# kartikmadhira1/YA_VO

Measured on AMD Instinct MI355X. Metric: frames/sec (detect+describe+match+PnP) on 1241×376 KITTI stereo; RMSE vs CPU ref, higher is better.
Workload: dtype u8

## Files before the change

ya_vo_amd/csrc/yavo_batch.hip:

```cpp
#include "yavo_host.h"

using namespace yavo;

namespace {

constexpr int kMaxTimedRuns = 4096;

int upload_pairs_rev(yv_batch* b) {
    if (!b->m2_alloc || b->n_pairs <= 0) return YV_OK;
    std::vector<int32_t> r(b->h_pairs.size());
    for (size_t i = 0; i + 1 < r.size(); i += 2) {
        r[i] = b->h_pairs[i + 1];
        r[i + 1] = b->h_pairs[i];
    }
    YV_HIP(hipMemcpyAsync(b->pairs_rev, r.data(), sizeof(int32_t) * r.size(), hipMemcpyHostToDevice, b->ctx->stream));
    YV_HIP(hipStreamSynchronize(b->ctx->stream));
    return YV_OK;
}

int record_stage(yv_batch* b, hipStream_t s, int run, int stage) {
    if (!b->timing || run < 0) return YV_OK;
    if (b->timing == 2 && stage > 1) return YV_OK;
    YV_HIP(hipEventRecord(b->events[(size_t)run * kEvPerRun + stage], s));
    return YV_OK;
}

yavo::MatchLists match_lists(const yv_batch* b) { return {b->desc, b->keypoints, b->kp_count, b->max_kp}; }

yavo::MatchRecords match_records(const yv_batch* b, bool deferred) {
    return {b->matches,  b->match_count, b->filtered, b->filt_count,
            b->match_dj, b->match_lim,   deferred ? b->match_pos : nullptr};
}

int ensure_match_pos(yv_batch* b) {
    if (b->match_pos) return YV_OK;
    return b->mem.alloc(&b->match_pos, (size_t)std::max(b->max_pairs, 1) * (size_t)b->max_kp);
}

static_assert(YV_SUBPIX_NONE == yavo::kSubpixNone && YV_SUBPIX_OK == yavo::kSubpixOk &&
                  YV_SUBPIX_OUTSIDE == yavo::kSubpixOutside && YV_SUBPIX_EDGE == yavo::kSubpixEdge,
              "yavo.h / yavo_internal.h");

int subpix_fill_none(yv_batch* b, hipStream_t s) {
    const size_t n = (size_t)std::max(b->max_pairs, 1) * (size_t)b->max_kp;
    YV_HIP(hipMemsetAsync(b->subpix_dcol, 0, n * sizeof(int32_t), s));
    YV_HIP(hipMemsetAsync(b->subpix_sad, 0xFF, n * sizeof(int32_t), s));
    YV_HIP(hipMemsetAsync(b->subpix_status, YV_SUBPIX_NONE, n, s));
    return YV_OK;
}

int ensure_subpix(yv_batch* b) {
    if (b->subpix_alloc) return YV_OK;
    const size_t nk = (size_t)b->max_kp, np = (size_t)std::max(b->max_pairs, 1);
    int rc = YV_OK;
    rc |= b->mem.alloc(&b->subpix_pairs, np);
    rc |= b->mem.alloc(&b->subpix_dcol, np * nk);
    rc |= b->mem.alloc(&b->subpix_sad, np * nk);
    rc |= b->mem.alloc(&b->subpix_status, np * nk);
    if (rc != YV_OK) {
        b->mem.release(b->subpix_pairs, b->subpix_dcol, b->subpix_sad, b->subpix_status);
        return YV_ERR_HIP;
    }
    b->subpix_alloc = true;
    return YV_OK;
}

}

namespace yavo {

void batch_free(yv_batch* b) {
    if (!b) return;
    if (b->bstream) (void)hipStreamSynchronize(b->bstream);
    if (b->side) (void)hipStreamSynchronize(b->side);
    if (b->rstream) (void)hipStreamSynchronize(b->rstream);
    if (b->lk) yv_lk_destroy(b->lk);
    delete b;
}

static_assert(YV_MATCH_RATIO == yavo::kMatchRatio && YV_MATCH_MUTUAL == yavo::kMatchMutual, "yavo.h / yavo_internal.h");
static_assert(sizeof(yv_match2) == sizeof(int4), "nn2 is written as int4 {d1, j1, d2, j2}");

bool match_filter_args_ok(int flags, int num, int den) {
    if (flags < 0 || flags > (YV_MATCH_RATIO | YV_MATCH_MUTUAL)) return false;
    if ((flags & YV_MATCH_RATIO) && !(num > 0 && num <= den && den <= 32768)) return false;
    return true;
}

int ensure_match2(yv_batch* b) {
    if (b->m2_alloc) return YV_OK;
    const size_t nk = (size_t)b->max_kp, np = (size_t)std::max(b->max_pairs, 1);
    int rc = YV_OK;
    rc |= b->mem.alloc(&b->match_key2, np * nk);
    rc |= b->mem.alloc(&b->rev_key, np * nk);
    rc |= b->mem.alloc(&b->pairs_rev, np * 2);
    rc |= b->mem.alloc(&b->nn2, np * nk);
    rc |= b->mem.alloc(&b->rev, np * nk);
    rc |= b->mem.alloc(&b->keep, np * nk);
    if (rc != YV_OK) {
        b->mem.release(b->match_key2, b->rev_key, b->pairs_rev, b->nn2, b->rev, b->keep);
        return YV_ERR_HIP;
    }
    hipStream_t s = b->ctx->stream;
    YV_HIP(hipMemsetAsync(b->match_key2, 0xFF, np * nk * sizeof(uint32_t), s));
    YV_HIP(hipMemsetAsync(b->rev_key, 0xFF, np * nk * sizeof(uint32_t), s));
    YV_HIP(hipMemsetAsync(b->nn2, 0, np * nk * sizeof(int4), s));
    YV_HIP(hipMemsetAsync(b->rev, 0xFF, np * nk * sizeof(int32_t), s));
    YV_HIP(hipMemsetAsync(b->keep, 0, np * nk, s));
    YV_HIP(hipStreamSynchronize(s));
    b->m2_alloc = true;
    return upload_pairs_rev(b);
}

bool gate_ok(const int32_t* g) {
    for (int k = 0; k < 4; ++k)
        if (g[k] < -yavo::kGateMaxCoord || g[k] > yavo::kGateMaxCoord) return false;
    return g[0] <= g[1] && g[2] <= g[3];
}

int ensure_gates(yv_batch* b, int max_row, int max_col) {
    if (b->gate_alloc) return YV_OK;
    const int n_bands = max_row / yavo::kGateBandRows + 1;
    int shift = 6;
    while (n_bands * ((max_col >> shift) + 1) > yavo::kGateMaxCells && shift < 16) ++shift;
    if (n_bands * ((max_col >> shift) + 1) > yavo::kGateMaxCells) return YV_ERR_CAPACITY;
    const size_t nk = (size_t)b->max_kp, np = (size_t)std::max(b->max_pairs, 1), ns = (size_t)b->nslots;
    int rc = YV_OK;
    rc |= b->mem.alloc(&b->gates, np * 4);
    rc |= b->mem.alloc(&b->gate_sorted, ns * nk);
    rc |= b->mem.alloc(&b->gate_band, ns * (size_t)(n_bands + 1));
    if (rc != YV_OK) {
        b->mem.release(b->gates, b->gate_sorted, b->gate_band);
        return YV_ERR_HIP;
    }
    b->gate_bands = n_bands;
    b->gate_cols = (max_col >> shift) + 1;
    b->gate_shift = shift;
    b->gate_alloc = true;
    return YV_OK;
}

bool select_fits(const yv_ctx* ctx, int H, int W) {
    if (ctx->sel_q <= 0) return true;
    const int64_t cy = (H + ctx->sel_rows - 1) / ctx->sel_rows, cx = (W + ctx->sel_cols - 1) / ctx->sel_cols;
    return cy * cx <= yavo::kSelMaxCells;
}

int ensure_select(yv_batch* b) {
    if (b->sel_alloc) return YV_OK;
    const size_t ni = (size_t)b->max_images;
    int rc = YV_OK;
    rc |= b->mem.alloc(&b->sel_keys, ni * (size_t)b->cap);
    rc |= b->mem.alloc(&b->sel_starts, ni * (size_t)(yavo::kSelMaxCells + 1));
    rc |= b->mem.alloc(&b->sel_counts, 3 * ni);
    if (rc != YV_OK) {
        b->mem.release(b->sel_keys, b->sel_starts, b->sel_counts);
        return YV_ERR_HIP;
    }
    b->sel_alloc = true;
    return YV_OK;
}

void launch_select_topk(yv_batch* b, int n_images, int keep, hipStream_t s) {
    const yv_ctx* ctx = b->ctx;
    uint32_t* count = b->cand_count;
    uint32_t* seen = b->cand_seen;
    if (select_on(ctx)) {
        count = yavo::launch_select(b->cand_keys, b->cap, b->cand_count, b->cand_seen, n_images, b->H, b->W,
                                    ctx->sel_radius, ctx->sel_rows, ctx->sel_cols, ctx->sel_q, b->sel_keys,
                                    b->sel_starts, b->sel_counts, s);
        seen = b->sel_counts + 2 * (size_t)b->max_images;
    }
    yavo::launch_topk(b->cand_keys, b->cap, count, seen, n_images, b->H, b->W, b->max_kp, keep, b->det_rc, b->det_resp,
                      b->det_count, b->kp_src, b->kp_count, b->kp_band, b->band_off, b->brief_heads, s);
}

int ensure_steer(yv_batch* b) {
    if (b->steer_alloc) return YV_OK;
    const size_t n = (size_t)b->nslots * (size_t)b->max_kp;
    int rc = YV_OK;
    rc |= b->mem.alloc(&b->steer_bin, n);
    rc |= b->mem.alloc(&b->steer_mom, 2 * n);
    if (rc != YV_OK) {
        b->mem.release(b->steer_bin, b->steer_mom);
        return YV_ERR_HIP;
    }
    hipStream_t s = b->ctx->stream;
    YV_HIP(hipMemsetAsync(b->steer_bin, 0, n, s));
    YV_HIP(hipMemsetAsync(b->steer_mom, 0, 2 * n * sizeof(int32_t), s));
    YV_HIP(hipStreamSynchronize(s));
    b->steer_alloc = true;
    return YV_OK;
}

void launch_describe(yv_batch* b, int n_images, int max_workers, hipStream_t s) {
    yv_ctx* ctx = b->ctx;
    if (steer_on(ctx)) {
        const yavo::SteerTables t{ctx->steer_bins, ctx->steer_radius, ctx->d_steer_dirs, ctx->d_steer_addr};
        yavo::launch_brief_steer(b->blur, n_images, b->H, b->W, t, b->kp_src, b->kp_count, b->max_kp, b->keypoints,
                                 b->desc, b->steer_bin, b->steer_mom, s);
        return;
    }
    const bool new_loff = b->loff_version != ctx->offsets_version;
    b->loff_version = ctx->offsets_version;
    yavo::launch_brief(b->blur, n_images, b->H, b->W, ctx->d_offsets, b->kp_src, b->kp_band, b->band_off, b->max_kp,
                       b->keypoints, b->desc, b->brief_loff, new_loff, b->brief_heads, max_workers, s);
}

int prepare_select(yv_batch* b, int H, int W) {
    if (!select_on(b->ctx)) return YV_OK;
    if (!select_fits(b->ctx, H, W)) return YV_ERR_CAPACITY;
    return ensure_select(b);
}

int match_stage(yv_batch* b, MatchStage st, hipStream_t s, int run) {
    const yavo::MatchLists lists = match_lists(b);
    uint32_t* key2 = st.top2 ? b->match_key2 : nullptr;
    if (st.gated) {
        yavo::launch_gate_sort(b->keypoints, b->kp_count, b->nslots, b->max_kp, b->gate_bands, b->gate_cols,
                               b->gate_shift, b->gate_sorted, b->gate_band, s);
        yavo::launch_match_gated(lists, b->pairs, st.n_pairs, b->gate_bands, b->gate_sorted, b->gate_band, b->gates,
                                 false, b->match_key, key2, s);
        if (st.with_rev)
            yavo::launch_match_gated(lists, b->pairs_rev, st.n_pairs, b->gate_bands, b->gate_sorted, b->gate_band,
                                     b->gates, true, b->rev_key, nullptr, s);
    } else {
        yavo::launch_match(lists, b->pairs, st.n_pairs, st.max_train, b->match_key, key2, s);
        if (st.with_rev) yavo::launch_match(lists, b->pairs_rev, st.n_pairs, st.max_train_rev, b->rev_key, nullptr, s);
    }
    const int rc = record_stage(b, s, run, 4);
    const yavo::FinalizeRobust rb{b->match_key2, b->rev_key, st.flags, st.num, st.den, b->nn2, b->rev, b->keep};
    const yavo::MatchRecords out = match_records(b, st.defer_records);
    yavo::launch_match_finalize(b->match_key, lists, b->pairs, st.n_pairs, st.thr, out, st.top2 ? &rb : nullptr, s,
                                st.kp_count_copy, st.n_slots);
    if (st.defer_records) {
        YV_HIP(hipEventRecord(b->ev_keys, s));
        YV_HIP(hipStreamWaitEvent(b->rstream, b->ev_keys, 0));
        yavo::launch_match_records({lists.desc, lists.keypoints, st.kp_count_copy, lists.max_kp}, b->pairs, st.n_pairs,
                                   out, records_workgroups(b->ctx), b->rstream);
        YV_HIP(hipEventRecord(b->ev_records, b->rstream));
        b->records_pending = true;
    }
    return rc;
}

}

extern "C" {

int yv_batch_create(yv_ctx* ctx, int max_images, int H, int W, int max_kp, int max_pairs, yv_batch** out) {
    if (!ctx || !out || max_images <= 0 || H < 9 || W < 9 || max_kp <= 0 || max_kp > yavo::kMaxKp ||
        max_pairs < 0 || (int64_t)H * W >= (1ll << 31))
        return YV_ERR_INVALID;
    if (W > yavo::kMaxWidth) return YV_ERR_CAPACITY;
    if (H > yavo::kBandRows * yavo::kMaxBands) return YV_ERR_CAPACITY;
    *out = nullptr;
    if (set_device(ctx) != YV_OK) return YV_ERR_HIP;
    yv_batch* b = new (std::nothrow) yv_batch();
    if (!b) return YV_ERR_INVALID;
    b->ctx = ctx;
    b->max_images = max_images;
    b->H = H;
    b->W = W;
    b->max_kp = max_kp;
    b->max_pairs = max_pairs;
    b->nslots = max_images + 1;
    b->cap = (int64_t)(H - 8) * (W - 8);
    const size_t ns = (size_t)b->nslots, nk = (size_t)max_kp, np = (size_t)std::max(max_pairs, 1);
    int rc = YV_OK;
    rc |= b->mem.alloc(&b->cand_keys, (size_t)max_images * (size_t)b->cap);
    rc |= b->mem.alloc(&b->cand_count, ns);
    rc |= b->mem.alloc(&b->cand_seen, ns);
    rc |= b->mem.alloc(&b->det_rc, ns * nk * 2);
    rc |= b->mem.alloc(&b->det_resp, ns * nk);
    rc |= b->mem.alloc(&b->det_count, ns);
    rc |= b->mem.alloc(&b->kp_src, ns * nk * 4);
    rc |= b->mem.alloc(&b->kp_count, ns);
    rc |= b->mem.alloc(&b->kp_count_build, ns);
    rc |= b->mem.alloc(&b->kp_band, ns * nk * 4);
    rc |= b->mem.alloc(&b->band_off, ns * (size_t)(yavo::kMaxBands + 1));
    rc |= b->mem.alloc(&b->brief_loff, 512);
    rc |= b->mem.alloc(&b->brief_heads, (size_t)yavo::kBriefHeads);
    rc |= b->mem.alloc(&b->keypoints, ns * nk);
    rc |= b->mem.alloc(&b->desc, ns * nk);
    rc |= b->mem.alloc(&b->blur, (size_t)max_images * (size_t)yavo::blur_image_bytes(H, W));
    rc |= b->mem.alloc(&b->pairs, np * 2);
    rc |= b->mem.alloc(&b->match_key, np * nk);
    rc |= b->mem.alloc(&b->matches, np * nk);
    rc |= b->mem.alloc(&b->match_count, np);
    rc |= b->mem.alloc(&b->filtered, np * nk);
    rc |= b->mem.alloc(&b->filt_count, np);
    rc |= b->mem.alloc(&b->match_dj, np * nk);
    rc |= b->mem.alloc(&b->match_lim, np);
    rc |= b->mem.alloc(&b->staging, (size_t)H * W);
    if (rc != YV_OK) {
        batch_free(b);
        return YV_ERR_HIP;
    }
    hipStream_t s = ctx->stream;
    bool ok = hipMemsetAsync(b->cand_count, 0, ns * sizeof(uint32_t), s) == hipSuccess &&
              hipMemsetAsync(b->cand_seen, 0, ns * sizeof(uint32_t), s) == hipSuccess &&
              hipMemsetAsync(b->kp_count, 0, ns * sizeof(int32_t), s) == hipSuccess &&
              hipMemsetAsync(b->det_count, 0, ns * sizeof(int32_t), s) == hipSuccess &&
              hipMemsetAsync(b->match_key, 0xFF, np * nk * sizeof(uint32_t), s) == hipSuccess &&
              hipMemsetAsync(b->keypoints, 0, ns * nk * sizeof(yv_keypoint), s) == hipSuccess &&
              hipMemsetAsync(b->match_count, 0, np * sizeof(int32_t), s) == hipSuccess &&
              hipMemsetAsync(b->filt_count, 0, np * sizeof(int32_t), s) == hipSuccess &&
              hipMemsetAsync(b->match_lim, 0, np * sizeof(int32_t), s) == hipSuccess &&
              hipStreamSynchronize(s) == hipSuccess;
    if (!ok) {
        batch_free(b);
        return YV_ERR_HIP;
    }
    *out = b;
    return YV_OK;
}

void yv_batch_destroy(yv_batch* b) {
    if (!b) return;
    (void)hipSetDevice(b->ctx->device);
    (void)hipStreamSynchronize(b->ctx->stream);
    batch_free(b);
}

int yv_batch_set_pairs(yv_batch* b, const int32_t* pairs, int n_pairs) {
    if (!b || n_pairs < 0 || n_pairs > b->max_pairs || (n_pairs > 0 && !pairs)) return YV_ERR_INVALID;
    for (int i = 0; i < 2 * n_pairs; ++i)
        if (pairs[i] < 0 || pairs[i] > b->max_images) return YV_ERR_INVALID;
    if (set_device(b->ctx) != YV_OK) return YV_ERR_HIP;
    if (b->bstream) YV_HIP(hipStreamSynchronize(b->bstream));
    b->build_pending = false;
    if (drain_records(b) != YV_OK) return YV_ERR_HIP;
    if (n_pairs > 0) {
        YV_HIP(hipMemcpyAsync(b->pairs, pairs, sizeof(int32_t) * 2 * (size_t)n_pairs, hipMemcpyHostToDevice,
                              b->ctx->stream));
        YV_HIP(hipStreamSynchronize(b->ctx->stream));
    }
    b->h_pairs.assign(pairs, pairs + 2 * (size_t)n_pairs);
    b->n_pairs = n_pairs;
    b->n_tracks = 0;
    b->gated = false;
    b->subpix_on = false;
    return upload_pairs_rev(b);
}

int yv_batch_set_stereo_subpix(yv_batch* b, const int32_t* pair_idx, int n, int half_win, int search, int flags) {
    if (!b || n < 0) return YV_ERR_INVALID;
    if (!pair_idx || n == 0) {
        b->subpix_on = false;
        return YV_OK;
    }
    if (half_win < 1 || half_win > yavo::kSubpixMaxWin || search < 1 || search > yavo::kSubpixMaxSearch || flags < 0 ||
        flags > YV_SUBPIX_DROP_EDGE || n > b->n_pairs)
        return YV_ERR_INVALID;
    std::vector<uint8_t> seen((size_t)b->n_pairs, 0);
    for (int i = 0; i < n; ++i) {
        const int p = pair_idx[i];
        if (p < 0 || p >= b->n_pairs || seen[p]) return YV_ERR_INVALID;
        if (b->h_pairs[2 * p] >= b->max_images || b->h_pairs[2 * p + 1] >= b->max_images) return YV_ERR_INVALID;
        seen[p] = 1;
    }
    if (set_device(b->ctx) != YV_OK) return YV_ERR_HIP;
    const int rc = ensure_subpix(b);
    if (rc != YV_OK) return rc;
    hipStream_t s = b->ctx->stream;
    YV_HIP(hipDeviceSynchronize());
    b->build_pending = false;
    YV_HIP(hipMemcpyAsync(b->subpix_pairs, pair_idx, sizeof(int32_t) * (size_t)n, hipMemcpyHostToDevice, s));
    if (subpix_fill_none(b, s) != YV_OK) return YV_ERR_HIP;
    YV_HIP(hipStreamSynchronize(s));
    b->subpix_n = n;
    b->subpix_win = half_win;
    b->subpix_search = search;
    b->subpix_flags = flags;
    b->subpix_on = true;
    return YV_OK;
}

int yv_batch_subpix_view_get(yv_batch* b, yv_batch_subpix_view* v) {
    if (!b || !v || !b->subpix_alloc) return YV_ERR_INVALID;
    v->dcol_q8 = b->subpix_dcol;
    v->sad = b->subpix_sad;
    v->status = b->subpix_status;
    return YV_OK;
}

int yv_batch_set_match_gates(yv_batch* b, const int32_t* gates, int n_pairs) {
    if (!b) return YV_ERR_INVALID;
    if (!gates || n_pairs == 0) {
        b->gated = false;
        return YV_OK;
    }
    if (n_pairs != b->n_pairs) return YV_ERR_INVALID;
    for (int p = 0; p < n_pairs; ++p)
        if (!gate_ok(gates + 4 * p)) return YV_ERR_INVALID;
    if (set_device(b->ctx) != YV_OK) return YV_ERR_HIP;
    const int rc = ensure_gates(b, b->H - 1, b->W - 1);
    if (rc != YV_OK) return rc;
    YV_HIP(hipStreamSynchronize(b->ctx->stream));
    YV_HIP(hipMemcpyAsync(b->gates, gates, sizeof(int32_t) * 4 * (size_t)n_pairs, hipMemcpyHostToDevice,
                          b->ctx->stream));
    YV_HIP(hipStreamSynchronize(b->ctx->stream));
    b->gated = true;
    return YV_OK;
}

int yv_batch_set_match_filter(yv_batch* b, int flags, int ratio_num, int ratio_den) {
    if (!match_filter_args_ok(flags, ratio_num, ratio_den) || !b) return YV_ERR_INVALID;
    if (flags != 0) {
        if (set_device(b->ctx) != YV_OK) return YV_ERR_HIP;
        const int rc = ensure_match2(b);
        if (rc != YV_OK) return rc;
    }
    b->match_flags = flags;
    b->ratio_num = (flags & YV_MATCH_RATIO) ? ratio_num : 0;
    b->ratio_den = (flags & YV_MATCH_RATIO) ? ratio_den : 1;
    return YV_OK;
}

int yv_batch_match2_view_get(yv_batch* b, yv_batch_match2_view* v) {
    if (!b || !v || !b->m2_alloc) return YV_ERR_INVALID;
    v->nn2 = reinterpret_cast<const yv_match2*>(b->nn2);
    v->rev = b->rev;
    v->keep = b->keep;
    return YV_OK;
}

int yv_batch_orient_view_get(yv_batch* b, yv_batch_orient_view* v) {
    if (!b || !v || !b->steer_alloc) return YV_ERR_INVALID;
    v->bin = b->steer_bin;
    v->moments = b->steer_mom;
    return YV_OK;
}

int yv_batch_enable_timing(yv_batch* b, int on) {
    if (!b) return YV_ERR_INVALID;
    if (on && b->events.empty()) {
        if (set_device(b->ctx) != YV_OK) return YV_ERR_HIP;
        b->events.resize((size_t)kMaxTimedRuns * kEvPerRun);
        for (auto& e : b->events) YV_HIP(b->mem.event(&e, hipEventDefault));
        b->tracked.assign(kMaxTimedRuns, 0);
    }
    b->timing = on == 2 ? 2 : (on != 0 ? 1 : 0);
    b->runs_recorded = 0;
    b->last_run = -1;
    std::fill(b->tracked.begin(), b->tracked.end(), 0);
    return YV_OK;
}

int yv_batch_stage_times(yv_batch* b, float* ms, int* n_runs) {
    if (!b || !ms) return YV_ERR_INVALID;
    for (int i = 0; i < 8; ++i) ms[i] = 0.f;
    const int runs = std::min(b->runs_recorded, kMaxTimedRuns);
    if (n_runs) *n_runs = runs;
    if (runs == 0) return YV_OK;
    for (int r = 0; r < runs; ++r) {
        const hipEvent_t* ev = &b->events[(size_t)r * kEvPerRun];
        if (b->timing == 2) {
            float t = 0.f;
            YV_HIP(hipEventSynchronize(ev[1]));
            YV_HIP(hipEventElapsedTime(&t, ev[0], ev[1]));
            ms[0] += t;
            continue;
        }
        YV_HIP(hipEventSynchronize(ev[b->tracked[r] ? 8 : 5]));
        for (int st = 0; st < 5; ++st) {
            float t = 0.f;
            YV_HIP(hipEventElapsedTime(&t, ev[st], ev[st + 1]));
            ms[st] += t;
        }
        if (b->tracked[r])
            for (int st = 5; st < 7; ++st) {
                float t = 0.f;
                YV_HIP(hipEventElapsedTime(&t, ev[st + 1], ev[st + 2]));
                ms[st] += t;
            }
    }
    return YV_OK;
}

int yv_batch_run(yv_batch* b, const uint8_t* d_images, int n_images, int stride, int64_t image_pitch, int match_thr,
                 int carry_from, void* stream) {
    if (!b || !d_images || n_images <= 0 || n_images > b->max_images || stride < b->W ||
        image_pitch < (int64_t)stride * (b->H - 1) + b->W || carry_from >= n_images)
        return YV_ERR_INVALID;
    yv_ctx* ctx = b->ctx;
    if (set_device(ctx) != YV_OK) return YV_ERR_HIP;
    hipStream_t s = stream ? reinterpret_cast<hipStream_t>(stream) : ctx->stream;
    const int H = b->H, W = b->W, K = b->max_kp;
    const int keep = std::min(ctx->max_corners, K);
    const int sel = prepare_select(b, H, W);
    if (sel != YV_OK) return sel;
    const bool steer = steer_on(ctx);
    if (steer && ensure_steer(b) != YV_OK) return YV_ERR_HIP;
    const bool defer_records = b->rstream && b->n_tracks > 0 && b->timing != 1;
    if (defer_records && ensure_match_pos(b) != YV_OK) return YV_ERR_HIP;
    if (b->pending_carry >= 0 && (join_build(b, s) != YV_OK || join_records(b, s) != YV_OK)) return YV_ERR_HIP;
    if (b->pending_carry >= 0) {
        const size_t c = (size_t)b->pending_carry, dst = (size_t)b->max_images, nk = (size_t)K;
        YV_HIP(hipMemcpyAsync(b->keypoints + dst * nk, b->keypoints + c * nk, nk * sizeof(yv_keypoint),
                              hipMemcpyDeviceToDevice, s));
        YV_HIP(hipMemcpyAsync(b->desc + dst * nk, b->desc + c * nk, nk * sizeof(Desc), hipMemcpyDeviceToDevice, s));
        YV_HIP(hipMemcpyAsync(b->kp_count + dst, b->kp_count + c, sizeof(int32_t), hipMemcpyDeviceToDevice, s));
        if (steer) {
            YV_HIP(hipMemcpyAsync(b->steer_bin + dst * nk, b->steer_bin + c * nk, nk, hipMemcpyDeviceToDevice, s));
            YV_HIP(hipMemcpyAsync(b->steer_mom + dst * nk * 2, b->steer_mom + c * nk * 2, nk * 2 * sizeof(int32_t),
                                  hipMemcpyDeviceToDevice, s));
        }
        b->pending_carry = -1;
// ... 90 lines not shown
```

ya_vo_amd/csrc/yavo_brief.hip:

```cpp
#include <hip/hip_runtime.h>
#include <stdint.h>

#include <algorithm>

#include "yavo_internal.h"
#include "yavo_wave.h"

namespace yavo {


constexpr int BR_BAND = kBandRows;
constexpr int BR_ROWS = BR_BAND + 17;
constexpr int BR_NT = 1024;
constexpr int BR_NW = BR_NT / 64;
static_assert(4 * BR_NT >= kMaxKp, "brief_kernel loads at most 4 * BR_NT band records");

__device__ __forceinline__ int brief_take(int32_t* heads, int label, int total, int& at) {
    const int q = total >> 3, r = total & 7;
    while (at < kBriefHeads) {
        const int x = (label + at) & 7;
        const int len = q + (x < r ? 1 : 0);
        if (len > 0) {
            const int v = atomicAdd(&heads[x], 1);
            if (v < len) return (x < r ? x * (q + 1) : r * (q + 1) + (x - r) * q) + v;
        }
        ++at;
    }
    return -1;
}

#ifdef YAVO_LM_PROFILE
constexpr int kBriefProfSlots = 16384;
__device__ unsigned long long g_brief_prof[kBriefProfSlots][6];
#define BP_DECL unsigned long long bp_acc[3] = {0, 0, 0}; unsigned long long bp_t = __builtin_readcyclecounter(); \
    unsigned long long bp_bands = 0; const unsigned long long bp_rt0 = __builtin_amdgcn_s_memrealtime();
#define BP_MARK(k) do { const unsigned long long t_ = __builtin_readcyclecounter(); bp_acc[k] += t_ - bp_t; bp_t = t_; } while (0)
#define BP_BAND() do { ++bp_bands; } while (0)
#define BP_STORE() do { \
        if (threadIdx.x == 0 && blockIdx.x < kBriefProfSlots) { \
            g_brief_prof[blockIdx.x][0] = bp_acc[0]; g_brief_prof[blockIdx.x][1] = bp_acc[1]; \
            g_brief_prof[blockIdx.x][2] = bp_rt0; \
            g_brief_prof[blockIdx.x][3] = __builtin_amdgcn_s_memrealtime(); \
            g_brief_prof[blockIdx.x][4] = (unsigned long long)__builtin_amdgcn_s_getreg(0xF804) | (bp_bands << 32); \
            g_brief_prof[blockIdx.x][5] = (unsigned long long)__builtin_amdgcn_s_getreg(0xF814) | (bp_acc[2] << 32); \
        } \
    } while (0)
#else
#define BP_DECL
#define BP_MARK(k) do {} while (0)
#define BP_BAND() do {} while (0)
#define BP_STORE() do {} while (0)
#endif

__global__ __launch_bounds__(BR_NT) __attribute__((amdgpu_waves_per_eu(8, 8))) void brief_kernel(
                                                    const uint8_t* __restrict__ blur, int H, int W,
                                                    const int32_t* __restrict__ kp_src,
                                                    const int32_t* __restrict__ kp_band,
                                                    const int32_t* __restrict__ band_off, int max_kp,
                                                    yv_keypoint* __restrict__ keypoints, Desc* __restrict__ desc,
                                                    const int2* __restrict__ loff, int32_t* __restrict__ heads,
                                                    int total) {
    extern __shared__ __attribute__((aligned(16))) uint8_t s_band[];
    uint32_t* s_list = reinterpret_cast<uint32_t*>(s_band + BR_ROWS * brief_lds_stride(W));
    int* s_next = reinterpret_cast<int*>(s_list + kMaxKp);
    BP_DECL
    const int nbands = (H + BR_BAND - 1) / BR_BAND;
    const int tid = threadIdx.x, lane = lane_id(), wave = __builtin_amdgcn_readfirstlane(tid >> 6);
    const int label = (int)blockIdx.x & 7;
    const int bp = blur_pitch(W), LS = brief_lds_stride(W);
    const int wpr = LS >> 4;
    const int nw = BR_ROWS * wpr;
    const int kw_fix = W >> 4;
    uint4* s4 = reinterpret_cast<uint4*>(s_band);
    typedef __attribute__((address_space(3))) void* lds_ptr_t;
    uint32_t pk[4];
#pragma unroll
    for (int u = 0; u < 4; ++u) {
        const int k = tid + u * BR_NT;
        const int j = k / wpr, q = k - j * wpr;
        pk[u] = k < nw ? (uint32_t)(j * bp + 16 * q) | ((uint32_t)j << 17) | (q == kw_fix ? 1u << 23 : 0u) | (1u << 24)
                       : 0u;
    }
    auto fetch_next = [&]() {
        int at = s_next[3];
        const int nl = brief_take(heads, label, total, at);
        s_next[3] = at;
        int nlo = 0, nn = 0;
        if (nl >= 0) {
            const int ni = nl / nbands;
            const int32_t* bo = band_off + (int64_t)ni * (kMaxBands + 1) + (nl - ni * nbands);
            nlo = bo[0];
            nn = bo[1] - nlo;
        }
        s_next[0] = nl;
        s_next[1] = nlo;
        s_next[2] = nn;
    };
    if (tid == BR_NT - 64) {
        s_next[3] = 0;
        fetch_next();
    }
    __syncthreads();
    int lb = __builtin_amdgcn_readfirstlane(s_next[0]);
    int klo = __builtin_amdgcn_readfirstlane(s_next[1]);
    int nbk = __builtin_amdgcn_readfirstlane(s_next[2]);
    BP_MARK(2);
    while (lb >= 0) {
        int t = tid;
        asm volatile("" : "+v"(t), "+v"(pk[0]), "+v"(pk[1]), "+v"(pk[2]), "+v"(pk[3]));
        const int img = lb / nbands;
        const int band = lb - img * nbands;
        const int r0 = band * BR_BAND, rb = r0 - 8;
        const int4* src = reinterpret_cast<const int4*>(kp_src) + (int64_t)img * max_kp;
        if (nbk > 0) {
            uint32_t z = 0u;
            asm volatile("" : "+v"(z));
#pragma unroll
            for (int u = 0; u < 4; ++u) {
                const int r = rb + (int)((pk[u] >> 17) & 63u);
                if ((pk[u] >> 24) != 0u && (r < 0 || r >= H)) s4[t + u * BR_NT] = make_uint4(z, z, z, z);
            }
            const int4* kb = reinterpret_cast<const int4*>(kp_band) + (int64_t)img * max_kp + klo;
            int4 kq[4];
#pragma unroll
            for (int u = 0; u < 4; ++u) {
                const int j = u * BR_NT + t;
                kq[u] = kb[j < nbk ? j : 0];
            }
            const uint8_t* b = blur + (int64_t)img * H * bp;
            const int64_t boff = (int64_t)rb * bp;
            uint32_t nx[4];
#pragma unroll
            for (int u = 0; u < 4; ++u) {
                const int r = rb + (int)((pk[u] >> 17) & 63u);
                nx[u] = 0u;
                if ((pk[u] >> 24) != 0u && r >= 0 && r < H) {
                    __builtin_amdgcn_global_load_lds(b + (boff + (int64_t)(pk[u] & 0x1FFFFu)),
                                                     (lds_ptr_t)(s4 + (t & ~63) + u * BR_NT), 16, 0, 0);
                    if ((pk[u] & (1u << 23)) != 0u && r + 1 < H) nx[u] = (uint32_t)b[(int64_t)(r + 1) * bp];
                }
            }
            __builtin_amdgcn_s_waitcnt(0);
#pragma unroll
            for (int u = 0; u < 4; ++u) asm volatile("" : "+v"(kq[u].x), "+v"(kq[u].y), "+v"(kq[u].w), "+v"(nx[u]));
#pragma unroll
            for (int u = 0; u < 4; ++u) {
                const int j = u * BR_NT + t;
                if (j < nbk)
                    s_list[j] = ((uint32_t)kq[u].w << 16) | ((uint32_t)kq[u].y << 5) | (uint32_t)(kq[u].x - r0);
            }
#pragma unroll
            for (int u = 0; u < 4; ++u) {
                const int r = rb + (int)((pk[u] >> 17) & 63u);
                if ((pk[u] >> 24) != 0u && (pk[u] & (1u << 23)) != 0u && r >= 0 && r < H)
                    s_band[16 * (t + u * BR_NT) + (W & 15)] = (uint8_t)nx[u];
            }
            const int sh_fix = 8 * (W & 3), dw_fix = (W >> 2) & 3;
            int wprw = wpr;
            asm volatile("" : "+s"(wprw));
            for (int k = t + 4 * BR_NT; k < nw; k += BR_NT) {
                const int j = k / wprw, q = k - j * wprw;
                const int r = rb + j;
                uint4 w = make_uint4(0, 0, 0, 0);
                if (r >= 0 && r < H) {
                    w = reinterpret_cast<const uint4*>(b + (int64_t)r * bp)[q];
                    if (q == kw_fix) {
                        const uint32_t nxx = r + 1 < H ? (uint32_t)b[(int64_t)(r + 1) * bp] : 0u;
                        const uint32_t m = ~(0xFFu << sh_fix);
                        if (dw_fix == 0) w.x = (w.x & m) | (nxx << sh_fix);
                        else if (dw_fix == 1) w.y = (w.y & m) | (nxx << sh_fix);
                        else if (dw_fix == 2) w.z = (w.z & m) | (nxx << sh_fix);
                        else w.w = (w.w & m) | (nxx << sh_fix);
                    }
                }
                s4[k] = w;
            }
        }
        __syncthreads();
        BP_MARK(0);
        BP_BAND();
        if (tid == BR_NT - 64) fetch_next();
        const int nb = nbk;
        if (nb > 0) {
            int ln = lane;
            asm volatile("" : "+v"(ln));
            uint8_t* rec_b = reinterpret_cast<uint8_t*>(keypoints + (int64_t)img * max_kp);
            Desc* d_base = desc + (int64_t)img * max_kp;
            const int G = (nb + 31) >> 5;
            const int nitems = ((32 * G + 63) >> 6) * 4;
            for (int item = wave; item < nitems; item += BR_NW) {
                const int g = item & 3, kd = (item >> 2) * 64 + ln;
                const int k = (kd & 31) * G + (kd >> 5);
                const bool act = (kd >> 5) < G && k < nb;
                const uint32_t e = s_list[act ? k : nb - 1];
                const int i = (int)(e >> 16), row = r0 + (int)(e & 31u), col = (int)((e >> 5) & 2047u);
                const int id = (act && g == 0) ? src[i].z : 0;
                const int la = (row - rb) * LS + col;
                const int2* lo = loff + 64 * g;
                uint32_t w[2] = {0u, 0u};
#pragma unroll 1
                for (int c = 7; c >= 0; --c) {
                    const int2* oc = lo + 8 * c;
                    uint32_t acc = w[c >> 2];
#pragma unroll
                    for (int j = 7; j >= 0; --j) {
                        const int2 o = oc[j];
                        const uint32_t p1 = s_band[la + o.x], p2 = s_band[la + o.y];
                        acc = __builtin_amdgcn_alignbit(acc, p2 - p1, 31);
                    }
                    if (c >= 4) w[1] = acc;
                    else w[0] = acc;
                }
                if (act) {
                    reinterpret_cast<uint2*>(d_base + i)[g] = make_uint2(w[0], w[1]);
                    uint8_t* r = rec_b + (int64_t)i * 48;
                    if (g == 0) {
                        reinterpret_cast<int32_t*>(r)[0] = row;
                        reinterpret_cast<int32_t*>(r)[1] = col;
                        reinterpret_cast<int32_t*>(r)[2] = id;
                        r[12] = 0;
                    }
                    r[13 + 8 * g] = (uint8_t)w[0];
                    *reinterpret_cast<uint16_t*>(r + 14 + 8 * g) = (uint16_t)(w[0] >> 8);
                    *reinterpret_cast<uint32_t*>(r + 16 + 8 * g) = (w[0] >> 24) | (w[1] << 8);
                    r[20 + 8 * g] = (uint8_t)(w[1] >> 24);
                    if (g == 3) {
                        r[45] = 0;
                        *reinterpret_cast<uint16_t*>(r + 46) = 0;
                    }
                }
                asm volatile("" ::"v"(id));
            }
        }
        BP_MARK(1);
        __builtin_amdgcn_fence(__ATOMIC_RELEASE, "workgroup", "local");
        __builtin_amdgcn_s_barrier();
        __builtin_amdgcn_fence(__ATOMIC_ACQUIRE, "workgroup", "local");
        lb = __builtin_amdgcn_readfirstlane(s_next[0]);
        klo = __builtin_amdgcn_readfirstlane(s_next[1]);
        nbk = __builtin_amdgcn_readfirstlane(s_next[2]);
        BP_MARK(2);
    }
    BP_STORE();
}

__global__ void brief_loff_kernel(const int8_t* __restrict__ offsets, int LS, int2* __restrict__ loff) {
    const int t = threadIdx.x;
    const int8_t* o = offsets + 4 * t;
    loff[t] = make_int2((int)o[0] * LS + (int)o[1], (int)o[2] * LS + (int)o[3]);
}

void launch_brief(const uint8_t* blur, int n_images, int H, int W, const int8_t* offsets, const int32_t* kp_src,
                  const int32_t* kp_band, const int32_t* band_off, int max_kp, yv_keypoint* keypoints, Desc* desc,
                  int32_t* loff, bool new_loff, int32_t* heads, int max_workers, hipStream_t s) {
    const int total = ((H + BR_BAND - 1) / BR_BAND) * n_images;
    dim3 grid(std::max(1, std::min(max_workers, total)));
    const size_t lds = brief_lds_bytes(W);
    int2* lo = reinterpret_cast<int2*>(loff);
    if (new_loff) hipLaunchKernelGGL(brief_loff_kernel, dim3(1), dim3(256), 0, s, offsets, brief_lds_stride(W), lo);
    hipLaunchKernelGGL(brief_kernel, grid, dim3(BR_NT), lds, s, blur, H, W, kp_src, kp_band, band_off, max_kp,
                       keypoints, desc, lo, heads, total);
}

__global__ void pack_desc_kernel(const yv_keypoint* __restrict__ keypoints, const int32_t* __restrict__ kp_count,
                                 int max_kp, Desc* __restrict__ desc) {
    const int slot = blockIdx.y;
    const int i = blockIdx.x * blockDim.x + threadIdx.x;
    if (i >= kp_count[slot] || i >= max_kp) return;
    const uint8_t* rec = reinterpret_cast<const uint8_t*>(keypoints + (int64_t)slot * max_kp + i);
    Desc d;
#pragma unroll
    for (int q = 0; q < 8; ++q) {
        d.w[q] = (uint32_t)rec[13 + 4 * q] | ((uint32_t)rec[14 + 4 * q] << 8) | ((uint32_t)rec[15 + 4 * q] << 16) |
                 ((uint32_t)rec[16 + 4 * q] << 24);
    }
    desc[(int64_t)slot * max_kp + i] = d;
}

void launch_pack_desc(const yv_keypoint* keypoints, const int32_t* kp_count, int n_slots, int max_kp, Desc* desc,
                      hipStream_t s) {
    dim3 grid((max_kp + 255) / 256, n_slots);
    hipLaunchKernelGGL(pack_desc_kernel, grid, dim3(256), 0, s, keypoints, kp_count, max_kp, desc);
}

}

#ifdef YAVO_LM_PROFILE
extern "C" int yv_debug_brief_prof(unsigned long long* out ) {
    return hipMemcpyFromSymbol(out, HIP_SYMBOL(yavo::g_brief_prof), sizeof(unsigned long long) * 16384 * 6) ==
                   hipSuccess ? 0 : -2;
}
#endif
```

ya_vo_amd/csrc/yavo_internal.h:

```cpp
#pragma once

#include <hip/hip_runtime.h>
#include <stdint.h>

#include "../../include/yavo/yavo_types.h"

struct yv_ctx;

namespace yavo {

__host__ __device__ inline double cube_cr(double t) {
    const double p = t * t, e1 = fma(t, t, -p);
    const double q = p * t, e2 = fma(p, t, -q);
    return q + (e2 + e1 * t);
}

constexpr int kMaxKp = 4096;
constexpr int kMaxWidth = 2048;
constexpr int kBandRows = 32;
constexpr int kMaxBands = 256;
constexpr int kBandCounters = 1024;
constexpr int kFastTileW = 64;
constexpr int kFastTileH = 56;
__host__ __device__ constexpr int blur_pitch(int W) { return (W + 1 + 127) & ~127; }
__host__ __device__ constexpr int brief_lds_stride(int W) { return (W + 1 + 15) & ~15; }
__host__ __device__ constexpr size_t brief_lds_bytes(int W) {
    return (size_t)(kBandRows + 17) * brief_lds_stride(W) + sizeof(uint32_t) * kMaxKp + 16;
}
constexpr int kBriefHeads = 8;
inline int brief_workers_per_cu(int W) { return brief_lds_bytes(W) <= 80 * 1024 ? 2 : 1; }
__host__ __device__ constexpr int64_t blur_image_bytes(int H, int W) { return (int64_t)H * blur_pitch(W); }
__device__ __forceinline__ int xcd_swizzle(int b, int nblocks) {
    const int q = nblocks >> 3, r = nblocks & 7, xcd = b & 7, slot = b >> 3;
    return (xcd < r ? xcd * (q + 1) : r * (q + 1) + (xcd - r) * q) + slot;
}

struct Desc {
    uint32_t w[8];
};
struct Mat3 {
    double v[9];
};

void launch_fast_harris(const uint8_t* imgs, int n_images, int H, int W, int stride, int64_t pitch,
                        int thr, int eig, uint64_t* cand_keys, int64_t cap, uint32_t* cand_count,
                        hipStream_t s);
void launch_detect_blur(const uint8_t* imgs, int n_images, int H, int W, int stride, int64_t pitch, int thr,
                        int eig, uint64_t* cand_keys, int64_t cap, uint32_t* cand_count, const uint16_t* k9_host,
                        uint8_t* blur, hipStream_t s);
void launch_blur9(const uint8_t* imgs, int n_images, int H, int W, int stride, int64_t pitch,
                  const uint16_t* k9_host, uint8_t* blur, hipStream_t s);
__device__ __forceinline__ uint64_t make_key(float resp, uint32_t idx) {
    if (resp == 0.0f) resp = 0.0f;
    uint32_t u = __float_as_uint(resp);
    uint32_t ord = (u & 0x80000000u) ? ~u : (u | 0x80000000u);
    return ((uint64_t)(~ord) << 32) | (uint64_t)idx;
}
__device__ __forceinline__ float key_resp(uint64_t key) {
    uint32_t ord = ~(uint32_t)(key >> 32);
    uint32_t u = (ord & 0x80000000u) ? (ord & 0x7fffffffu) : ~ord;
    return __uint_as_float(u);
}

constexpr int kSelMaxCells = 8192;
constexpr int kSelTileRows = 32, kSelTileCols = 64;
constexpr int kSelMaxRadius = 8;
constexpr int kSelMaxPerCell = 4096;
constexpr int kSelMinCell = 8, kSelMaxCell = 8192;
uint32_t* launch_select(uint64_t* cand_keys, int64_t cap, uint32_t* cand_count, uint32_t* cand_seen, int n_images,
                        int H, int W, int nms_radius, int cell_rows, int cell_cols, int per_cell, uint64_t* scratch,
                        int32_t* starts, uint32_t* counts, hipStream_t s);

void launch_topk(const uint64_t* cand_keys, int64_t cap, uint32_t* cand_count, uint32_t* cand_seen, int n_images,
                 int H, int W, int max_kp, int keep, int32_t* det_rc, float* det_resp, int32_t* det_count,
                 int32_t* kp_src, int32_t* kp_count, int32_t* kp_band, int32_t* band_off, int32_t* brief_heads,
                 hipStream_t s);
void launch_kp_boundary(const int32_t* det_rc, const int32_t* det_count, int n_images, int H, int W,
                        int max_kp, int32_t* kp_src, int32_t* kp_count, int32_t* kp_band, int32_t* band_off,
                        int32_t* brief_heads, hipStream_t s);

void launch_brief(const uint8_t* blur, int n_images, int H, int W, const int8_t* offsets,
                  const int32_t* kp_src, const int32_t* kp_band, const int32_t* band_off, int max_kp,
                  yv_keypoint* keypoints, Desc* desc, int32_t* loff, bool new_loff, int32_t* heads, int max_workers,
                  hipStream_t s);
void launch_pack_desc(const yv_keypoint* keypoints, const int32_t* kp_count, int n_slots, int max_kp,
                      Desc* desc, hipStream_t s);
constexpr int kSteerMaxBins = 64;
constexpr int kSteerMaxRadius = 15;
constexpr int kSteerMaxDir = 256;
constexpr int kSteerPatchStride = 40;
struct SteerTables {
    int n_bins, radius;
    const int16_t* dirs;
    const uint32_t* taddr;
};
void steer_pack_offsets(const int8_t* offsets, int n_tests, uint32_t* out);
void launch_brief_steer(const uint8_t* blur, int n_images, int H, int W, const SteerTables& t, const int32_t* kp_src,
                        const int32_t* kp_count, int max_kp, yv_keypoint* keypoints, Desc* desc, uint8_t* bin,
                        int32_t* moments, hipStream_t s);
void launch_orient(const uint8_t* blur, int H, int W, const SteerTables& t, const int32_t* rc, const int32_t* count,
                   int max_kp, uint8_t* bin, int32_t* moments, hipStream_t s);

struct MatchLists {
    const Desc* desc;
    const yv_keypoint* keypoints;
    const int32_t* kp_count;
    int max_kp;
};
void launch_match(const MatchLists& lists, const int32_t* pairs, int n_pairs, int max_train, uint32_t* match_key,
                  uint32_t* match_key2, hipStream_t s);
constexpr int kGateBandRows = 32;
constexpr int kGateMaxCells = 8192;
constexpr int kGateMaxCoord = 65535;
void launch_gate_sort(const yv_keypoint* keypoints, const int32_t* kp_count, int n_slots, int max_kp, int n_bands,
                      int col_cells, int col_shift, uint2* sorted, int32_t* band_start, hipStream_t s);
void launch_match_gated(const MatchLists& lists, const int32_t* pairs, int n_pairs, int n_bands, const uint2* sorted,
                        const int32_t* band_start, const int32_t* gates, bool mirror, uint32_t* match_key,
                        uint32_t* match_key2, hipStream_t s);

struct MatchRecords {
    yv_match* matches;
    int32_t* match_count;
    yv_match* filtered;
    int32_t* filt_count;
    int2* match_dj;
    int32_t* match_lim;
    int32_t* match_pos;
};
constexpr int kMatchRatio = 1, kMatchMutual = 2;
struct FinalizeRobust {
    uint32_t* match_key2;
    uint32_t* rev_key;
    int flags, num, den;
    int4* nn2;
    int32_t* rev;
    uint8_t* keep;
};
void launch_match_finalize(uint32_t* match_key, const MatchLists& lists, const int32_t* pairs, int n_pairs, int thr,
                           const MatchRecords& out, const FinalizeRobust* rb, hipStream_t s,
                           int32_t* kp_count_copy = nullptr, int n_slots = 0);
void launch_match_records(const MatchLists& lists, const int32_t* pairs, int n_pairs, const MatchRecords& out,
                          int max_workgroups, hipStream_t s);
void launch_filter_records(const yv_match* in, int n, int thr, yv_match* out, int32_t* out_count,
                           hipStream_t s);

constexpr int kSubpixNone = 0, kSubpixOk = 1, kSubpixOutside = 2, kSubpixEdge = 3;
constexpr int kSubpixMaxWin = 7, kSubpixMaxSearch = 8;
struct SubpixOut {
    int32_t* dcol_q8;
    int32_t* sad;
    uint8_t* status;
};
void launch_subpix_list(const uint8_t* left, const uint8_t* right, int H, int W, int stride, const yv_match* m, int n,
                        int half_win, int search, const SubpixOut& out, hipStream_t s);
void launch_subpix_batch(const uint8_t* images, int n_images, int H, int W, int stride, int64_t pitch,
                         const int32_t* marked, int n_marked, const int32_t* pairs, const yv_keypoint* keypoints,
                         const int32_t* kp_count, const int2* match_dj, const int32_t* match_lim,
                         const uint8_t* keep, int max_kp, int half_win, int search, const SubpixOut& out,
                         hipStream_t s);

size_t f_ransac_ws_bytes(int n_lists, int iters);
void launch_f_ransac(const yv_match* matches, int64_t list_stride, const int32_t* counts, int n_lists,
                     const int32_t* samples, int64_t sample_stride, int iters, double thr, double* F_out,
                     int32_t* max_inliers, int32_t* found, void* ws, hipStream_t s);
void launch_triangulate(const yv_match* m, int n, const double* poses2, const double* K, double* Xw, uint8_t* ok,
                        int32_t* n_ok, hipStream_t s, const int32_t* dcol_q8 = nullptr);
void launch_world2camera(const double* X, int n, const double* T, const double* K, double* out, hipStream_t s);

void launch_pose_lm(const int32_t* offsets, int n_problems, const double* X, const double* uv, const double* K,
                    double* poses, uint8_t* outlier, int32_t* inliers, hipStream_t s);
void launch_pose_gn(const int32_t* offsets, int n_problems, const double* X, const double* uv, const double* K,
                    double* poses, int32_t* iters, hipStream_t s);
void launch_track_pose(int n_tracks, const int32_t* edge_count, int stride, const double* edge_X,
                       const double* edge_uv, const double* K, const double* priors, double* poses,
                       uint8_t* edge_outlier, int32_t* inliers, hipStream_t s);

struct TrackSrc {
    const int32_t* pairs;
    const yv_keypoint* keypoints;
    const int32_t* kp_count;
    const int2* match_dj;
    const int32_t* match_lim;
    int max_kp;
    const double* K;
    const double* T_right;
    const uint8_t* keep;
    const int32_t* sub_dcol;
    const uint8_t* sub_status;
    bool drop_edge;
};
struct EdgeOut {
    double* X;
    double* uv;
    int32_t* query;
    int32_t* count;
};
struct PointsOut {
    double* X;
    float* pts;
    int32_t* query;
    int32_t* count;
};
void launch_track_build(const int32_t* tracks, int n_tracks, const TrackSrc& src, const EdgeOut& out, hipStream_t s);
void launch_stereo_points(const int32_t* stereo_pairs, int n_tracks, const TrackSrc& src, const PointsOut& out,
                          hipStream_t s);
void launch_lk_edges(int n_tracks, const PointsOut& pts, const float* next, const uint8_t* status, int max_kp,
                     const EdgeOut& out, hipStream_t s);

constexpr int kLkMaxLevels = 8;
struct LkParams {
    int levels = 0, win = 11, max_count = 30;
    double eps2 = 1e-4, min_eig = 1e-3;
    int h[kLkMaxLevels] = {}, w[kLkMaxLevels] = {};
    int ps[kLkMaxLevels] = {}, ds[kLkMaxLevels] = {};
    int64_t off[kLkMaxLevels] = {};
    const uint8_t* img0 = nullptr;
    int stride0 = 0;
    int64_t pitch0 = 0;
    uint8_t* pyr = nullptr;
    int64_t pyr_pitch = 0;
    int16_t* der = nullptr;
    int64_t der_pitch = 0;
};
void launch_lk_pyramid(const LkParams& P, int n_images, hipStream_t s);
void launch_lk_derivs(const LkParams& P, int image, int level, int16_t* der, hipStream_t s);
void launch_lk_track(const LkParams& P, const int32_t* pairs, int n_pairs, const float* pts, const int32_t* counts,
                     int pts_stride, int max_pts, float* next_pts, uint8_t* status, float* err, hipStream_t s);

constexpr int kEssChunk = 64;
constexpr int kEssChunkWide = 1024;
constexpr int kEssWidePairs = 8;
inline int ess_chunk_for(int max_pairs) { return max_pairs <= kEssWidePairs ? kEssChunkWide : kEssChunk; }
struct EssParams {
    int max_pairs = 0, max_points = 0, max_iters = 0;
    int chunk = kEssChunk;
    double* m1 = nullptr;
    double* m2 = nullptr;
    int32_t* idx = nullptr;
    double* models = nullptr;
    int32_t* nmod = nullptr;
    int32_t* good = nullptr;
    int32_t* state = nullptr;
    double* best = nullptr;
    double* cand = nullptr;
    int32_t* cgood = nullptr;
    uint64_t* rng_tab = nullptr;
    int rng_len = 0;
};
struct EssRun {
    double focal, ppx, ppy, prob, threshold;
    int max_iters;
};
void launch_find_essential(const EssParams& P, const EssRun& r, const float* pts1, const float* pts2,
                           const int32_t* counts, int n_pairs, int pts_stride, double* E, uint8_t* mask,
                           int32_t* found, int32_t* stats, hipStream_t s);
int launch_debug_ess_models(const EssParams& P, const double* q1, const double* q2, int n_sets, double* models,
                            int32_t* nmod, hipStream_t s);
void launch_recover_pose(const EssParams& P, const double* E, const float* pts1, const float* pts2,
                         const int32_t* counts, int n_pairs, int pts_stride, const Mat3& K, double* R, double* t,
                         int32_t* good, hipStream_t s);

namespace ba {
constexpr int kNT = 256;
constexpr int kTicketGroups = 64;
constexpr int kWLeaves = 4096;
constexpr int kWG = 16;
constexpr int kWLanes = kWLeaves / kWG;
}
struct BaParams {
    int P = 0, nf = 0, np = 0, ns = 0, L = 0, E = 0;
    const int32_t* ep = nullptr;
    const int32_t* el = nullptr;
    const double* meas = nullptr;
    const int32_t* pe_off = nullptr;
    const int32_t* pe = nullptr;
    const int32_t* le_off = nullptr;
    const int32_t* le = nullptr;
    const int32_t* cv_off = nullptr;
    const int32_t* cv_e1 = nullptr;
    const int32_t* cv_e2 = nullptr;
    double* poses = nullptr;
    double* X = nullptr;
    double* err = nullptr;
    double* Jp = nullptr;
    double* Jl = nullptr;
    double* Hpp = nullptr;
    double* bp = nullptr;
    double* Hll = nullptr;
    double* bl = nullptr;
    double* S = nullptr;
    double* bs = nullptr;
    double* xp = nullptr;
    double* xl = nullptr;
    int32_t* tr = nullptr;
    double* scal = nullptr;
    const int* gate = nullptr;
    const double* lam = nullptr;
    double* poses2 = nullptr;
    double* X2 = nullptr;
    int* cur = nullptr;
    struct BaCtl* ctl = nullptr;
    double* log = nullptr;
    unsigned long long* maxdiag = nullptr;
    unsigned* ticket = nullptr;
    double* part = nullptr;
    double* spart = nullptr;
    unsigned* sticket = nullptr;
    double* rpart = nullptr;
    unsigned* rticket = nullptr;
};
struct BaCtl {
    double currentChi, lambda, ni, rho;
    int q, it, stop, iters;
    int skip_iter, skip_trial, suspended, iter_done;
};
void launch_ba_linearize(const BaParams& P, const Mat3& K, int first, hipStream_t s);
void launch_ba_trial(const BaParams& P, const Mat3& K, double lambda, hipStream_t s);
void launch_ba_chi2(const BaParams& P, const Mat3& K, hipStream_t s);
void launch_ba_finish(const BaParams& P, hipStream_t s);
void launch_ba_ctl_resume(BaCtl* c, hipStream_t s);
void launch_ba_ldlt(const BaParams& P, hipStream_t s);

void launch_map_chunk(const double* rel, int n, int64_t first_frame, int kf_every, const int32_t* edge_count,
                      const double* edge_X, const uint8_t* edge_outlier, int max_kp, int max_kf, void* block,
                      hipStream_t s);

enum : int32_t {
    kPngOk = 0, kPngErrHeader = 1, kPngErrBlock = 2, kPngErrCode = 3, kPngErrOverrun = 4, kPngErrShort = 5,
    kPngErrFilter = 6, kPngErrCrc = 7, kPngErrAdler = 8,
    kPngErrFile = 9
};
struct PngPiece {
    int64_t src, dst;
    int32_t len, img;
};
void launch_png_gather(const uint8_t* src, uint8_t* dst, const PngPiece* pieces, int n, int32_t* crc_bad, hipStream_t s);
void launch_png_inflate(const uint8_t* src, const int64_t* off, const int32_t* len, int n, uint8_t* out,
                        int64_t out_pitch, uint32_t out_len, int32_t* status, int32_t* crc_bad, uint32_t* adler,
                        hipStream_t s);
void launch_png_unfilter(const uint8_t* raw, int64_t raw_pitch, int n, int H, int W, uint8_t* dst, int64_t dst_pitch,
                         int dst_stride, int32_t* status, const uint32_t* adler, uint32_t* bad_total, hipStream_t s);

int ctx_device(struct ::yv_ctx* ctx);
hipStream_t ctx_stream(struct ::yv_ctx* ctx);

}
```

Measured before the change: 265,500.

## Write keypoint headers at band load and keep BRIEF offsets in registers

The keypoint header (row, col, id) is now written once per keypoint while the band list is built, using the kp_band record that is already loaded. This removes the separate gather from kp_src in the descriptor loop and the g==0 store branch there. The inner BRIEF loop now holds each wave's test-offset group in a 16-int vector register, prefetches the next chunk, and issues 16 raw LDS byte loads per chunk through computed LDS addresses instead of reloading int2 offsets from global memory. The gain depends on each wave keeping a fixed group (relies on BR_NW%4==0), and the change raises VGPR pressure under the fixed waves-per-eu constraint. It also assumes kp_band's z field carries the id.

```diff
diff --git a/ya_vo_amd/csrc/yavo_batch.hip b/ya_vo_amd/csrc/yavo_batch.hip
--- a/ya_vo_amd/csrc/yavo_batch.hip
+++ b/ya_vo_amd/csrc/yavo_batch.hip
@@ -203,8 +203,8 @@
     }
     const bool new_loff = b->loff_version != ctx->offsets_version;
     b->loff_version = ctx->offsets_version;
-    yavo::launch_brief(b->blur, n_images, b->H, b->W, ctx->d_offsets, b->kp_src, b->kp_band, b->band_off, b->max_kp,
-                       b->keypoints, b->desc, b->brief_loff, new_loff, b->brief_heads, max_workers, s);
+    yavo::launch_brief(b->blur, n_images, b->H, b->W, ctx->d_offsets, b->kp_band, b->band_off, b->max_kp, b->keypoints,
+                       b->desc, b->brief_loff, new_loff, b->brief_heads, max_workers, s);
 }
 
 int prepare_select(yv_batch* b, int H, int W) {
diff --git a/ya_vo_amd/csrc/yavo_brief.hip b/ya_vo_amd/csrc/yavo_brief.hip
--- a/ya_vo_amd/csrc/yavo_brief.hip
+++ b/ya_vo_amd/csrc/yavo_brief.hip
@@ -54,7 +54,6 @@
 
 __global__ __launch_bounds__(BR_NT) __attribute__((amdgpu_waves_per_eu(8, 8))) void brief_kernel(
                                                     const uint8_t* __restrict__ blur, int H, int W,
-                                                    const int32_t* __restrict__ kp_src,
                                                     const int32_t* __restrict__ kp_band,
                                                     const int32_t* __restrict__ band_off, int max_kp,
                                                     yv_keypoint* __restrict__ keypoints, Desc* __restrict__ desc,
@@ -111,7 +110,6 @@
         const int img = lb / nbands;
         const int band = lb - img * nbands;
         const int r0 = band * BR_BAND, rb = r0 - 8;
-        const int4* src = reinterpret_cast<const int4*>(kp_src) + (int64_t)img * max_kp;
         if (nbk > 0) {
             uint32_t z = 0u;
             asm volatile("" : "+v"(z));
@@ -137,17 +135,25 @@
                 if ((pk[u] >> 24) != 0u && r >= 0 && r < H) {
                     __builtin_amdgcn_global_load_lds(b + (boff + (int64_t)(pk[u] & 0x1FFFFu)),
                                                      (lds_ptr_t)(s4 + (t & ~63) + u * BR_NT), 16, 0, 0);
-                    if ((pk[u] & (1u << 23)) != 0u && r + 1 < H) nx[u] = (uint32_t)b[(int64_t)(r + 1) * bp];
+                    if ((pk[u] & (1u << 23)) != 0u && r + 1 < H) nx[u] = (uint32_t)b[(r + 1) * bp];
                 }
             }
             __builtin_amdgcn_s_waitcnt(0);
 #pragma unroll
-            for (int u = 0; u < 4; ++u) asm volatile("" : "+v"(kq[u].x), "+v"(kq[u].y), "+v"(kq[u].w), "+v"(nx[u]));
+            for (int u = 0; u < 4; ++u)
+                asm volatile("" : "+v"(kq[u].x), "+v"(kq[u].y), "+v"(kq[u].z), "+v"(kq[u].w), "+v"(nx[u]));
+            uint8_t* rec_h = reinterpret_cast<uint8_t*>(keypoints + (int64_t)img * max_kp);
 #pragma unroll
             for (int u = 0; u < 4; ++u) {
                 const int j = u * BR_NT + t;
-                if (j < nbk)
+                if (j < nbk) {
                     s_list[j] = ((uint32_t)kq[u].w << 16) | ((uint32_t)kq[u].y << 5) | (uint32_t)(kq[u].x - r0);
+                    uint8_t* r = rec_h + (int64_t)kq[u].w * 48;
+                    reinterpret_cast<int32_t*>(r)[0] = kq[u].x;
+                    reinterpret_cast<int32_t*>(r)[1] = kq[u].y;
+                    reinterpret_cast<int32_t*>(r)[2] = kq[u].z;
+                    r[12] = 0;
+                }
             }
 #pragma unroll
             for (int u = 0; u < 4; ++u) {
@@ -188,38 +194,46 @@
             Desc* d_base = desc + (int64_t)img * max_kp;
             const int G = (nb + 31) >> 5;
             const int nitems = ((32 * G + 63) >> 6) * 4;
+            typedef int int16v __attribute__((ext_vector_type(16)));
+            typedef __attribute__((address_space(3))) const uint8_t* lds_u8_t;
+            static_assert(BR_NW % 4 == 0, "a wave keeps its test group over its items");
+            const int16v* lo = reinterpret_cast<const int16v*>(loff + 64 * (wave & 3));
+            int16v oc = lo[7];
             for (int item = wave; item < nitems; item += BR_NW) {
                 const int g = item & 3, kd = (item >> 2) * 64 + ln;
                 const int k = (kd & 31) * G + (kd >> 5);
                 const bool act = (kd >> 5) < G && k < nb;
                 const uint32_t e = s_list[act ? k : nb - 1];
                 const int i = (int)(e >> 16), row = r0 + (int)(e & 31u), col = (int)((e >> 5) & 2047u);
-                const int id = (act && g == 0) ? src[i].z : 0;
-                const int la = (row - rb) * LS + col;
-                const int2* lo = loff + 64 * g;
-                uint32_t w[2] = {0u, 0u};
+                const uint32_t la = (uint32_t)(uintptr_t)(lds_u8_t)(s_band + ((row - rb) * LS + col));
+                uint32_t w[2];
+#pragma unroll
+                for (int h = 1; h >= 0; --h) {
+                    uint32_t acc = 0u;
 #pragma unroll 1
-                for (int c = 7; c >= 0; --c) {
-                    const int2* oc = lo + 8 * c;
-                    uint32_t acc = w[c >> 2];
-#pragma unroll
-                    for (int j = 7; j >= 0; --j) {
-                        const int2 o = oc[j];
-                        const uint32_t p1 = s_band[la + o.x], p2 = s_band[la + o.y];
-                        acc = __builtin_amdgcn_alignbit(acc, p2 - p1, 31);
+                    for (int c = 4 * h + 3; c >= 4 * h; --c) {
+                        uint32_t p[16];
+#pragma unroll
+                        for (int q = 0; q < 16; ++q) p[q] = la + (uint32_t)oc[q];
+                        int cn = (c + 7) & 7;
+                        asm volatile("" : "+v"(p[0]), "+v"(p[1]), "+v"(p[2]), "+v"(p[3]), "+v"(p[4]), "+v"(p[5]),
+                                          "+v"(p[6]), "+v"(p[7]), "+v"(p[8]), "+v"(p[9]), "+v"(p[10]), "+v"(p[11]),
+                                          "+v"(p[12]), "+v"(p[13]), "+v"(p[14]), "+v"(p[15]), "+s"(cn));
+                        oc = lo[cn];
+#pragma unroll
+                        for (int q = 0; q < 16; ++q) p[q] = *(lds_u8_t)(uintptr_t)p[q];
+                        asm volatile("" : "+v"(p[0]), "+v"(p[1]), "+v"(p[2]), "+v"(p[3]), "+v"(p[4]), "+v"(p[5]),
+                                          "+v"(p[6]), "+v"(p[7]), "+v"(p[8]), "+v"(p[9]), "+v"(p[10]), "+v"(p[11]),
+                                          "+v"(p[12]), "+v"(p[13]), "+v"(p[14]), "+v"(p[15]), "+s"(oc));
+#pragma unroll
+                        for (int j = 7; j >= 0; --j)
+                            acc = __builtin_amdgcn_alignbit(acc, p[2 * j + 1] - p[2 * j], 31);
                     }
-                    if (c >= 4) w[1] = acc;
-                    else w[0] = acc;
+                    w[h] = acc;
                 }
                 if (act) {
                     reinterpret_cast<uint2*>(d_base + i)[g] = make_uint2(w[0], w[1]);
                     uint8_t* r = rec_b + (int64_t)i * 48;
-                    if (g == 0) {
-                        reinterpret_cast<int32_t*>(r)[0] = row;
-                        reinterpret_cast<int32_t*>(r)[1] = col;
-                        reinterpret_cast<int32_t*>(r)[2] = id;
-                        r[12] = 0;
-                    }
                     r[13 + 8 * g] = (uint8_t)w[0];
                     *reinterpret_cast<uint16_t*>(r + 14 + 8 * g) = (uint16_t)(w[0] >> 8);
                     *reinterpret_cast<uint32_t*>(r + 16 + 8 * g) = (w[0] >> 24) | (w[1] << 8);
@@ -229,7 +243,6 @@
                         *reinterpret_cast<uint16_t*>(r + 46) = 0;
                     }
                 }
-                asm volatile("" ::"v"(id));
             }
         }
         BP_MARK(1);
@@ -250,16 +263,16 @@
     loff[t] = make_int2((int)o[0] * LS + (int)o[1], (int)o[2] * LS + (int)o[3]);
 }
 
-void launch_brief(const uint8_t* blur, int n_images, int H, int W, const int8_t* offsets, const int32_t* kp_src,
-                  const int32_t* kp_band, const int32_t* band_off, int max_kp, yv_keypoint* keypoints, Desc* desc,
-                  int32_t* loff, bool new_loff, int32_t* heads, int max_workers, hipStream_t s) {
+void launch_brief(const uint8_t* blur, int n_images, int H, int W, const int8_t* offsets, const int32_t* kp_band,
+                  const int32_t* band_off, int max_kp, yv_keypoint* keypoints, Desc* desc, int32_t* loff, bool new_loff,
+                  int32_t* heads, int max_workers, hipStream_t s) {
     const int total = ((H + BR_BAND - 1) / BR_BAND) * n_images;
     dim3 grid(std::max(1, std::min(max_workers, total)));
     const size_t lds = brief_lds_bytes(W);
     int2* lo = reinterpret_cast<int2*>(loff);
     if (new_loff) hipLaunchKernelGGL(brief_loff_kernel, dim3(1), dim3(256), 0, s, offsets, brief_lds_stride(W), lo);
-    hipLaunchKernelGGL(brief_kernel, grid, dim3(BR_NT), lds, s, blur, H, W, kp_src, kp_band, band_off, max_kp,
-                       keypoints, desc, lo, heads, total);
+    hipLaunchKernelGGL(brief_kernel, grid, dim3(BR_NT), lds, s, blur, H, W, kp_band, band_off, max_kp, keypoints,
+                       desc, lo, heads, total);
 }
 
 __global__ void pack_desc_kernel(const yv_keypoint* __restrict__ keypoints, const int32_t* __restrict__ kp_count,
diff --git a/ya_vo_amd/csrc/yavo_internal.h b/ya_vo_amd/csrc/yavo_internal.h
--- a/ya_vo_amd/csrc/yavo_internal.h
+++ b/ya_vo_amd/csrc/yavo_internal.h
@@ -79,10 +79,9 @@
                         int max_kp, int32_t* kp_src, int32_t* kp_count, int32_t* kp_band, int32_t* band_off,
                         int32_t* brief_heads, hipStream_t s);
 
-void launch_brief(const uint8_t* blur, int n_images, int H, int W, const int8_t* offsets,
-                  const int32_t* kp_src, const int32_t* kp_band, const int32_t* band_off, int max_kp,
-                  yv_keypoint* keypoints, Desc* desc, int32_t* loff, bool new_loff, int32_t* heads, int max_workers,
-                  hipStream_t s);
+void launch_brief(const uint8_t* blur, int n_images, int H, int W, const int8_t* offsets, const int32_t* kp_band,
+                  const int32_t* band_off, int max_kp, yv_keypoint* keypoints, Desc* desc, int32_t* loff, bool new_loff,
+                  int32_t* heads, int max_workers, hipStream_t s);
 void launch_pack_desc(const yv_keypoint* keypoints, const int32_t* kp_count, int n_slots, int max_kp,
                       Desc* desc, hipStream_t s);
 constexpr int kSteerMaxBins = 64;
```

Result: no change. 267,400, median of 6 (+0.7%).
